# ariana-spalter/human-robot-gym

Hardware: AMD Instinct MI355X
Metric: env steps/sec (whole node), ReachHuman+shield 4096 envs (higher is better)
Workload: dtype f64

## Files before the change

### human-robot-gym_amd/csrc/hrgym_device.h

```cpp
#pragma once
#include <hip/hip_runtime.h>
#include <stdint.h>

#include "../../include/hrgym.h"
#include "../../include/hrgym_state.h"

#define NV HRG_NV
#define NARM HRG_NARM
#ifndef HRG_BOX
#define HRG_BOX 0
#endif
#ifndef HRG_LIFT
#define HRG_LIFT 0
#endif
#ifndef HRG_HANDOVER
#define HRG_HANDOVER 0
#endif
#ifndef HRG_STACK
#define HRG_STACK 0
#endif
#ifndef HRG_HULLS
#define HRG_HULLS 0
#endif
#ifndef HRG_HAMMER
#define HRG_HAMMER 0
#endif
#define HRG_BASE_TU (!HRG_BOX && !HRG_STACK && !HRG_HAMMER && !HRG_HULLS)
#define HRG_POSE_TABLE ((!HRG_BOX && !HRG_STACK && !HRG_HAMMER) || HRG_LIFT)
#define HRG_POSE_HCAP 0
#define HRG_POSE_SITE (6 * HRG_NHB)
#define HRG_POSE_ROOT (HRG_POSE_SITE + 3 * HRG_NHJ)
#define HRG_POSE_DIM (HRG_POSE_ROOT + 3)
#define NVT HRG_NVT
#if HRG_HAMMER
#define NVS HRG_NV_HAMMER
#define NCON_DYN HRG_NCON_DYN_HAMMER
#define HM_OB NV
#define HM_ON (NV + 6)
#define HM_OH (NV + 8)
#elif HRG_STACK
#define NVS HRG_NV_STACK
#define NCON_DYN HRG_NCON_DYN_STACK
#define NCUBE HRG_NCUBE
#elif HRG_BOX
#define NVS NVT
#define NCON_DYN HRG_NCON_DYN_BOX
#else
#define NVS NV
#define NCON_DYN HRG_NCON_DYN
#endif
#define BODY_BOX 100
#define DI __device__ __forceinline__
#ifndef HRG_MIN_WAVES
#define HRG_MIN_WAVES 4
#endif
#ifndef HRG_PHASE
#define HRG_PHASE __device__ __forceinline__
#endif
#define PH_DYNTERMS HRG_PHASE
#define PH_HUMAN HRG_PHASE
#define PH_SHIELD HRG_PHASE
#define PH_COLLIDE HRG_PHASE
#define PH_CLASSIFY HRG_PHASE
#define PH_DYNSTEP HRG_PHASE
#define HRG_PI 3.14159265358979323846
#define SIXTH (1.0 / 6.0)

#define GEOM_HUMAN0 HRG_NRCAP
#define GEOM_TABLE (HRG_NRCAP + HRG_NHB)
#define GEOM_FLOOR (GEOM_TABLE + 1)
#define GEOM_BOX (GEOM_FLOOR + 1)

#ifdef HRG_STAMPS
static __device__ unsigned long long g_stamps[32];
static __device__ unsigned long long g_stamps_slow[34];
static __device__ unsigned long long g_slow_thresh = ~0ull;
static __device__ unsigned long long g_envcyc[16384][3];
static __device__ unsigned long long g_envacc[16384][32];
__shared__ unsigned long long g_tbeg;
__shared__ unsigned long long g_acc[32];
__shared__ unsigned long long g_t0;
#define STAMP_NOW(var) do { __builtin_amdgcn_sched_barrier(0); asm volatile("s_memtime %0\n\ts_waitcnt lgkmcnt(0)" : "=s"(var) :: "memory"); __builtin_amdgcn_sched_barrier(0); } while (0)
#define STAMP_DECL
#define STAMP_INIT(lane) do { if ((lane) < 32) g_acc[lane] = 0; unsigned long long _t; STAMP_NOW(_t); g_t0 = _t; g_tbeg = _t; __syncthreads(); } while (0)
#define STAMP(k) do { unsigned long long _t; STAMP_NOW(_t); if (threadIdx.x == 0) { g_acc[k] += _t - g_t0; g_t0 = _t; } } while (0)
#define STAMP_FLUSH(lane)
#define COUNT(k, n) do { if (threadIdx.x == 0) g_acc[k] += (n); } while (0)
#define STAMP_FINAL(lane) do { __syncthreads(); if ((lane) < 32) atomicAdd(&g_stamps[lane], g_acc[lane]); { unsigned long long _te; STAMP_NOW(_te); if (_te - g_tbeg > g_slow_thresh) { if ((lane) < 32) atomicAdd(&g_stamps_slow[lane], g_acc[lane]); if ((lane) == 32) atomicAdd(&g_stamps_slow[32], 1ull); if ((lane) == 33) atomicAdd(&g_stamps_slow[33], _te - g_tbeg); } } if ((lane) < 32 && blockIdx.x < 16384) g_envacc[blockIdx.x][lane] = g_acc[lane]; if ((lane) == 0 && blockIdx.x < 16384) { unsigned long long _t; STAMP_NOW(_t); g_envcyc[blockIdx.x][0] = g_tbeg; g_envcyc[blockIdx.x][1] = _t; unsigned _hw, _xcc; asm volatile("s_getreg_b32 %0, hwreg(HW_REG_HW_ID)\n\ts_getreg_b32 %1, hwreg(HW_REG_XCC_ID)" : "=s"(_hw), "=s"(_xcc)); g_envcyc[blockIdx.x][2] = ((unsigned long long)_xcc << 32) | _hw; } } while (0)
#else
#define STAMP_DECL
#define STAMP_INIT(lane)
#define STAMP(k)
#define STAMP_FLUSH(lane)
#define COUNT(k, n)
#define STAMP_FINAL(lane)
#endif

struct DevModel {
  hrg_model_desc m;
  double Rbase[9];
  double Rq[NV][9];
  int32_t anc_mask[NV];
  int32_t hb_maxdepth;
  double sol_K, sol_Bd;
  double rcap_hl[HRG_NRCAP], hcap_hl[HRG_NHB];
  int32_t hb_njump;
  int32_t hb_jump[4][HRG_NHB];
  int32_t phase_mask;
  hrg_path brake_full;
  double brake_T, brake_ds;
  int32_t hc_n;
  int32_t hc_kind[HRG_NHCAP_MAX], hc_j1[HRG_NHCAP_MAX], hc_j2[HRG_NHCAP_MAX];
  double hc_th[HRG_NHCAP_MAX], hc_v[HRG_NHCAP_MAX], hc_a[HRG_NHCAP_MAX], hc_len[HRG_NHCAP_MAX];
  int32_t n_self;
  int32_t self_i[64], self_j[64];
  int32_t n_chk;
  int32_t chk_i[32], chk_j[32];
  hrg_clip_table clips;
  const double* pose_tab;
  const double* hull_dev;
  double hull_cen[HRG_NHULL][3];
  unsigned long long* mpr_fallback;
};

static inline void hull_centroids(const double* verts, const int32_t* off, double cen[HRG_NHULL][3]) {
  for (int h = 0; h < HRG_NHULL; h++) {
    double s[3] = {0, 0, 0};
    for (int i = off[h]; i < off[h + 1]; i++) for (int a = 0; a < 3; a++) s[a] += verts[3 * i + a];
    for (int a = 0; a < 3; a++) cen[h][a] = s[a] / (double)(off[h + 1] - off[h]);
  }
}

struct Contact {
  int32_t g1, g2, b1, b2;
  double dist, n[3], pos[3];
};

#define ROW_CON0 24
#define ROW_WELD0 (ROW_CON0 + 4 * NCON_DYN)
#if HRG_HAMMER
#define HROW_NFRIC 8
#define HROW_LIM0 9
#define HROW_NLIM 25
#define HROW_EQ0 27
#define HROW_CON0 36
#define HROW_NEQ 9
#define NROW 128
#elif HRG_STACK
#define SROW_WELD0 24
#define SROW_CON0 36
#define NROW HRG_NROW_STACK
#elif HRG_BOX && (HRG_HANDOVER || HRG_LIFT)
#define NROW (ROW_WELD0 + 6)
#else
#define NROW ROW_WELD0
#endif

struct GjkLds { double y[4][3], a[4][3], b[4][3], l[4], lam[4]; int ia[4], ib[4]; };
#define HRG_HULL_MPR (HRG_HULLS && (HRG_BOX || HRG_STACK || HRG_HAMMER))
#if HRG_HULL_MPR
struct MprLds { double v[5][3], a[5][3], b[5][3]; };
#endif
struct Lds {
  hrg_env_state st;
  double kR[NV][9], kp[NV][3], Sw[NV][3], Sv[NV][3], vw[NV][3], vv[NV][3];
  double M[NV * NV];
  double bias[NV], a0[NVS], Ma0[NVS], ctrl[NV], qacc[NVS], g[NVS], d[NVS];
#if HRG_BOX
  hrg_box_state bx;
  double bR[9];
  double bMr[9];
  double hand_q[4], hand_off[3];
  int palm_hit, palm_pad;
#if HRG_HANDOVER
  double hcap_keep[HRG_NHB][6];
#endif
#endif
  double act[NV];
  int acc_has_collision, acc_collision_type, acc_failsafe, acc_pad;
#if HRG_HAMMER
  hrg_hammer_state hm;
  double gR[2][9];
  double gc[HRG_HM_NGEOM][3];
  double nail_org[3], nail_axis[3];
  double Mb[64], fb[8];
  double Ihw[9], tauh[3];
  double nsG[(9 + 2 * NCON_DYN) * (10 + 2 * NCON_DYN) / 2];
  Contact con[NCON_DYN];
#elif HRG_STACK
  hrg_stack_state sk;
  Contact con[NCON_DYN];
#elif HRG_BOX
  Contact con[NCON_DYN];
#else
  Contact con[NCON_DYN];
#endif
  union {
    struct {
      double cq[NARM], cv[NARM], ca[NARM], qe[NARM];
      double scap[2][HRG_NSHIELD_RCAP][6];
      double rc[HRG_NSHIELD_RCAP][7];
      hrg_ltt cand;
    };
    struct {
      double F[NV][6];
    };
    struct {
      double hcap[HRG_NHB][6], rcapw[HRG_NRCAP][6];
      int hnear[HRG_NHB];
      double rcen[HRG_NRCAP][3];
#if HRG_HULL_MPR
      union { GjkLds gjk; MprLds mpr; };
#elif HRG_HULLS
      GjkLds gjk;
#endif
#if HRG_STACK
      double cR[NCUBE][9];
#endif
    };
#if HRG_HAMMER
    struct {
      double Jc[4 * NCON_DYN + HROW_NEQ][NVS + 1], rg[NROW], rh[NROW];
    };
#elif HRG_STACK
    struct {
      double Jc[4 * NCON_DYN][21], rg[NROW], rh[NROW];
      int con_ca[NCON_DYN], con_cb[NCON_DYN], con_rob[NCON_DYN + 1];
    };
#else
    struct {
      double Jc[4 * NCON_DYN + (HRG_LIFT ? 6 : 0)][NVS + 1], rg[NROW], rh[NROW];
    };
#endif
  };
};

#ifndef HRG_WG_WAVES
#define HRG_WG_WAVES 1
#endif
#if HRG_WG_WAVES > 1
__shared__ Lds g_Lw[HRG_WG_WAVES];
#define g_L (g_Lw[__builtin_amdgcn_readfirstlane((int)(threadIdx.x >> 6))])
#else
__shared__ Lds g_L;
#endif
DI int hrg_lane() { return (int)(threadIdx.x & 63u); }
#define HRG_FAIR_SLOTS (8 * 8 * 2 * 16 * 4 * 8)
struct StepOrder { int32_t* buf; int32_t n; int32_t parity; int32_t* fair; };
DI int hrg_env() { return (int)blockIdx.x * HRG_WG_WAVES + (int)(threadIdx.x >> 6); }
#define HRG_LAUNCH_DIMS(n) dim3(((n) + HRG_WG_WAVES - 1) / HRG_WG_WAVES), dim3(64 * HRG_WG_WAVES)

typedef const DevModel __attribute__((address_space(4)))* ModelPtr;
DI ModelPtr uniform_model(const DevModel* dm) {
  const unsigned long long a = (unsigned long long)dm;
  unsigned lo = __builtin_amdgcn_readfirstlane((unsigned)(a & 0xffffffffull));
  unsigned hi = __builtin_amdgcn_readfirstlane((unsigned)(a >> 32));
  asm volatile("" : "+s"(lo), "+s"(hi));
  return (ModelPtr)(((unsigned long long)hi << 32) | lo);
}

DI double fsqrt(double x) {
  const double y = __builtin_amdgcn_rsq(x);
  double g = x * y, h = 0.5 * y;
  const double r = __builtin_fma(-h, g, 0.5);
  g = __builtin_fma(g, r, g);
  h = __builtin_fma(h, r, h);
  g = __builtin_fma(__builtin_fma(-g, g, x), h, g);
  g = __builtin_fma(__builtin_fma(-g, g, x), h, g);
  return x > 0 ? g : 0.0;
}
DI void v3set(double* r, double a, double b, double c) { r[0] = a; r[1] = b; r[2] = c; }
template <class PA>
DI void v3cpy(double* r, PA a) { r[0] = a[0]; r[1] = a[1]; r[2] = a[2]; }
template <class PA, class PB>
DI void v3add(double* r, PA a, PB b) { r[0] = a[0] + b[0]; r[1] = a[1] + b[1]; r[2] = a[2] + b[2]; }
template <class PA, class PB>
DI void v3sub(double* r, PA a, PB b) { r[0] = a[0] - b[0]; r[1] = a[1] - b[1]; r[2] = a[2] - b[2]; }
template <class PA>
DI void v3scl(double* r, PA a, double s) { r[0] = a[0] * s; r[1] = a[1] * s; r[2] = a[2] * s; }
template <class PA, class PB>
DI void v3madd(double* r, PA a, PB b, double s) { r[0] = a[0] + b[0] * s; r[1] = a[1] + b[1] * s; r[2] = a[2] + b[2] * s; }
template <class PA, class PB>
DI double v3dot(PA a, PB b) { return a[0] * b[0] + a[1] * b[1] + a[2] * b[2]; }
template <class PA>
DI double v3norm(PA a) { return fsqrt(v3dot(a, a)); }
template <class PA, class PB>
DI void v3cross(double* r, PA a, PB b) {
  double x = a[1] * b[2] - a[2] * b[1], y = a[2] * b[0] - a[0] * b[2], z = a[0] * b[1] - a[1] * b[0];
  r[0] = x; r[1] = y; r[2] = z;
}
template <class PA, class PB>
DI void m3mulv(double* r, PA M, PB v) {
  double x = M[0] * v[0] + M[1] * v[1] + M[2] * v[2];
  double y = M[3] * v[0] + M[4] * v[1] + M[5] * v[2];
  double z = M[6] * v[0] + M[7] * v[1] + M[8] * v[2];
  r[0] = x; r[1] = y; r[2] = z;
}
template <class PA, class PB>
DI void m3mul(double* R, PA A, PB B) {
  double T[9];
#pragma unroll
  for (int i = 0; i < 3; i++)
#pragma unroll
    for (int j = 0; j < 3; j++) T[3 * i + j] = A[3 * i] * B[j] + A[3 * i + 1] * B[3 + j] + A[3 * i + 2] * B[6 + j];
#pragma unroll
  for (int i = 0; i < 9; i++) R[i] = T[i];
}
template <class PA>
DI void quat2mat(double* M, PA q) {
  double w = q[0], x = q[1], y = q[2], z = q[3];
  M[0] = 1 - 2 * (y * y + z * z); M[1] = 2 * (x * y - w * z); M[2] = 2 * (x * z + w * y);
  M[3] = 2 * (x * y + w * z); M[4] = 1 - 2 * (x * x + z * z); M[5] = 2 * (y * z - w * x);
  M[6] = 2 * (x * z - w * y); M[7] = 2 * (y * z + w * x); M[8] = 1 - 2 * (x * x + y * y);
}
template <class PA, class PB>
DI void quatmul(double* r, PA a, PB b) {
  double w = a[0] * b[0] - a[1] * b[1] - a[2] * b[2] - a[3] * b[3];
  double x = a[0] * b[1] + a[1] * b[0] + a[2] * b[3] - a[3] * b[2];
  double y = a[0] * b[2] - a[1] * b[3] + a[2] * b[0] + a[3] * b[1];
  double z = a[0] * b[3] + a[1] * b[2] - a[2] * b[1] + a[3] * b[0];
  r[0] = w; r[1] = x; r[2] = y; r[3] = z;
}
DI void sincos_small(double x, double* sn, double* cs) {
  const double k = rint(x * 6.36619772367581382433e-01);
  const double r = (x - k * 1.57079632673412561417e+00) - k * 6.07710050650619224932e-11;
  const double z = r * r;
  const double ps = r + r * z * (-1.66666666666666324348e-01 + z * (8.33333333332248946124e-03 + z * (-1.98412698298579493134e-04 +
                    z * (2.75573137070700676789e-06 + z * (-2.50507602534068634195e-08 + z * 1.58969099521155010221e-10)))));
  const double pc = 1.0 - 0.5 * z + z * z * (4.16666666666666019037e-02 + z * (-1.38888888888741095749e-03 + z * (2.48015872894767294178e-05 +
                    z * (-2.75573143513906633035e-07 + z * (2.08757232129817482790e-09 + z * -1.13596475577881948265e-11)))));
  const int q = ((int)k) & 3;
  const double s0 = (q & 1) ? pc : ps, c0 = (q & 1) ? ps : pc;
  *sn = (q & 2) ? -s0 : s0;
  *cs = ((q + 1) & 2) ? -c0 : c0;
}
template <class PA>
DI void axisangle2mat(double* M, PA ax, double ang) {
  double s, c;
  sincos_small(ang, &s, &c);
  double t = 1 - c, x = ax[0], y = ax[1], z = ax[2];
  M[0] = t * x * x + c; M[1] = t * x * y - s * z; M[2] = t * x * z + s * y;
  M[3] = t * x * y + s * z; M[4] = t * y * y + c; M[5] = t * y * z - s * x;
  M[6] = t * x * z - s * y; M[7] = t * y * z + s * x; M[8] = t * z * z + c;
}
DI double clampd(double x, double lo, double hi) { return x < lo ? lo : (x > hi ? hi : x); }

template <int CTRL, int ROW_MASK>
DI double dpp_f64(double v) {
  const long long b = __double_as_longlong(v);
  const int lo = __builtin_amdgcn_update_dpp(0, (int)(b & 0xffffffffLL), CTRL, ROW_MASK, 0xf, false);
  const int hi = __builtin_amdgcn_update_dpp(0, (int)(b >> 32), CTRL, ROW_MASK, 0xf, false);
  return __longlong_as_double(((long long)hi << 32) | (unsigned int)lo);
}
DI double wave_sum(double v) {
  v += dpp_f64<0xB1, 0xf>(v);
  v += dpp_f64<0x4E, 0xf>(v);
  v += dpp_f64<0x141, 0xf>(v);
  v += dpp_f64<0x140, 0xf>(v);
  v += dpp_f64<0x142, 0xa>(v);
  v += dpp_f64<0x143, 0xc>(v);
  const long long b = __double_as_longlong(v);
  const int lo = __builtin_amdgcn_readlane((int)(b & 0xffffffffLL), 63);
  const int hi = __builtin_amdgcn_readlane((int)(b >> 32), 63);
  return __longlong_as_double(((long long)hi << 32) | (unsigned int)lo);
}
DI double wave_max(double v) {
#pragma unroll
  for (int o = 32; o > 0; o >>= 1) { double t = __shfl_xor(v, o, 64); v = t > v ? t : v; }
  return v;
}
DI double row16_max(double v) {
  double t;
  t = dpp_f64<0xB1, 0xf>(v); v = t > v ? t : v;
  t = dpp_f64<0x4E, 0xf>(v); v = t > v ? t : v;
  t = dpp_f64<0x141, 0xf>(v); v = t > v ? t : v;
  t = dpp_f64<0x140, 0xf>(v); v = t > v ? t : v;
  return v;
}
#if HRG_WG_WAVES > 1
DI void wave_sync() { __builtin_amdgcn_fence(__ATOMIC_RELEASE, "workgroup"); __builtin_amdgcn_wave_barrier(); __builtin_amdgcn_fence(__ATOMIC_ACQUIRE, "workgroup"); }
#else
DI void wave_sync() { __syncthreads(); }
#endif

DI uint64_t mix64(uint64_t x) {
  x += 0x9E3779B97F4A7C15ULL;
  x = (x ^ (x >> 30)) * 0xBF58476D1CE4E5B9ULL;
  x = (x ^ (x >> 27)) * 0x94D049BB133111EBULL;
  return x ^ (x >> 31);
}
DI double rng_u01(uint64_t seed, uint64_t env, uint64_t episode, uint64_t stream, uint64_t idx) {
  uint64_t h = mix64(seed);
  h = mix64(h ^ (env * 0xD1B54A32D192ED03ULL));
  h = mix64(h ^ (episode * 0x8CB92BA72F3D8DD7ULL));
  h = mix64(h ^ (stream * 0xABC98388FB8FAC03ULL + idx));
  return (double)(h >> 11) * (1.0 / 9007199254740992.0);
}
// ... 486 lines not shown
```

### human-robot-gym_amd/csrc/hrgym_kernels.h

```cpp
#pragma once
#include "hrgym_device.h"
#if HRG_HULLS
#include "hrgym_hull.h"
#endif

DI void robot_chain_fk(const DevModel* __restrict__ dm_, int lane, bool shield_on) {
  const ModelPtr dm = uniform_model(dm_);
  Lds& L = g_L;
  double* sc = &L.rc[0][0];
  if (lane < 3 * NARM && (lane >= 2 * NARM || shield_on)) {
    const int cfg = lane / NARM, i = lane - NARM * cfg;
    const double q = cfg == 0 ? L.cq[i] : (cfg == 1 ? L.qe[i] : L.st.qpos[i]);
    double sn, cs;
    sincos_small(q, &sn, &cs);
    sc[2 * lane] = sn; sc[2 * lane + 1] = cs;
  }
  wave_sync();
  if (lane < 9 && (lane >= 6 || shield_on)) {
    const auto& m = dm->m;
    const int cfg = lane / 3, row = lane - 3 * cfg;
    double r0 = dm->Rbase[3 * row], r1 = dm->Rbase[3 * row + 1], r2 = dm->Rbase[3 * row + 2];
    double p = m.base_pos[row];
#pragma unroll 1
    for (int i = 0; i < NARM; i++) {
// ... 283 lines not shown
  Lds& L = g_L;
  hrg_env_state& s = L.st;
  const double* e = dm->pose_tab + f * HRG_POSE_DIM;
  const bool cap = lane < HRG_NHB, site = !cap && lane < HRG_NHB + HRG_NHJ;
  double y[6] = {0, 0, 0, 0, 0, 0};
  if (cap) {
    const double2* p = (const double2*)(e + HRG_POSE_HCAP + 6 * lane);
    const double2 a = p[0], b = p[1], d = p[2];
    y[0] = a.x; y[1] = a.y; y[2] = b.x; y[3] = b.y; y[4] = d.x; y[5] = d.y;
  } else if (site) {
    const double* p = e + HRG_POSE_SITE + 3 * (lane - HRG_NHB);
    y[0] = p[0]; y[1] = p[1]; y[2] = p[2];
  }
  const double __attribute__((address_space(4)))* ec = (const double __attribute__((address_space(4)))*)(e + HRG_POSE_ROOT);
  double R[9], o[3], x[3];
  quat2mat(R, s.human_rot_offset);
  v3add(o, s.human_pos_offset, ec);
  m3mulv(x, R, y);
  if (cap) {
    v3add(&L.hcap[lane][0], o, x);
    m3mulv(x, R, y + 3);
    v3add(&L.hcap[lane][3], o, x);
  } else if (site) v3add(L.st.human_site[lane - HRG_NHB], o, x);
  wave_sync();
}

DI void human_pose_fk(const DevModel* __restrict__ dm_, int lane, int clip, int at, int hold_body = -1, int hold_left = 0) {
  const ModelPtr dm = uniform_model(dm_);
#if HRG_POSE_TABLE
  (void)hold_body; (void)hold_left;
  human_pose_from_table(dm, lane, (int64_t)dm->clips.clip_offset[clip] + at);
#else
  Lds& L = g_L;
  hrg_env_state& s = L.st;
  const double* fr = dm->clips.frames + (dm->clips.clip_offset[clip] + at) * HRG_FRAME_DIM;
  double qbi[4], qa[4], c[3], mp[3], mq[4], q1[4];
  human_root(dm, clip, fr, c, qbi, qa);
  v3add(mp, c, s.human_pos_offset);
  quatmul(q1, s.human_rot_offset, qbi);
  quatmul(mq, q1, qa);
  human_fk_lanes(dm_, lane, mp, mq, fr + 7, hold_body, hold_left);
#endif
}

#if HRG_BOX || HRG_STACK || HRG_HAMMER
DI double loop_prop(ModelPtr dm, int64_t gid, int episode, int ai, int clip, int k, int speed) {
  double base = speed ? dm->clips.clip_loop_speed[clip][k % HRG_MAX_LOOP] : dm->clips.clip_loop_amp[clip][k % HRG_MAX_LOOP];
  if (k >= HRG_MAX_LOOP) base = speed ? dm->clips.clip_loop2_speed[clip][k - HRG_MAX_LOOP] : dm->clips.clip_loop2_amp[clip][k - HRG_MAX_LOOP];
  const double sf = speed ? dm->clips.clip_loop_speed_std[clip] : dm->clips.clip_loop_amp_std[clip];
  const double z = clampd(rng_gauss(dm->m.seed, (uint64_t)gid, (uint64_t)episode, STREAM_LOOP, (uint64_t)((ai * 2 * HRG_MAX_LOOP + k) * 2 + speed)), -3.0, 3.0);
  return base * exp(z * log(sf));
}
DI double layered_sines(ModelPtr dm, int64_t gid, int episode, int ai, int clip, int kfirst, int n, double t, double start) {
  static_assert(2 * HRG_MAX_LOOP <= 64, "one lane per loop property");
  const int lane = hrg_lane(), kk = lane % HRG_MAX_LOOP, sp = (lane / HRG_MAX_LOOP) & 1;
  const double mine = loop_prop(dm, gid, episode, ai, clip, kfirst + (kk < n ? kk : 0), sp);
  double sum = 0;
  for (int k = 0; k < n; k++) {
    const double A = __shfl(mine, k), S = __shfl(mine, HRG_MAX_LOOP + k);
    sum += A * sin((t - start) / (A / S)) + start;
  }
  return sum - start * (double)(n - 1);
}
#endif

PH_HUMAN void human_control(const DevModel* __restrict__ dm_, int lane, int64_t gid) {
  const ModelPtr dm = uniform_model(dm_);
  Lds& L = g_L;
  const auto& m = dm->m;
  hrg_env_state& s = L.st;
  int control_time = (int)floor((double)s.low_level_time / m.anim_step_length);
  int at = control_time - s.anim_start_time;
  int anim_index = s.anim_index, anim_start = s.anim_start_time;
  int clip = clip_of(dm, gid, s.episode, anim_index);
#if HRG_BOX
  if (m.task == HRG_TASK_INSPECTION) {
    hrg_box_state& bx = L.bx;
    const int classic = control_time - s.anim_start_time, k0 = dm->clips.clip_keyframes[clip][0], k1 = dm->clips.clip_keyframes[clip][1], len = dm->clips.clip_len[clip];
    int phase = bx.task_phase, nd = bx.n_delayed;
    at = classic;
    if (at > k0 && phase == HRG_PHASE_APPROACH) phase = HRG_PHASE_READY;
    if (phase == HRG_PHASE_READY) {
      const int nl = dm->clips.clip_n_loop[clip];
      double sum = 0;
      for (int k = 0; k < nl; k++) {
        const double A = loop_prop(dm, gid, s.episode, s.anim_index, clip, k, 0), S = loop_prop(dm, gid, s.episode, s.anim_index, clip, k, 1);
        sum += A * sin((double)(classic - k0) / (A / S)) + (double)k0;
      }
      at = (int)(sum - (double)k0 * (double)(nl - 1));
      nd = classic - at;
    } else at -= nd;
    if (at > k1) phase = HRG_PHASE_RETREAT;
    if (at >= len - 1) { phase = HRG_PHASE_COMPLETE; at = len - 1; }
    if (at < 0) at = 0;
    wave_sync();
    bx.task_phase = phase; bx.n_delayed = nd;
    if (lane < 3) bx.target[lane] = dm->clips.clip_target_pos[clip][lane] + s.human_pos_offset[lane];
  }
  int hold_body = -1, hold_left = 0;
#if HRG_HANDOVER
  if (m.task == HRG_TASK_HANDOVER_H2R) {
    hrg_box_state& bx = L.bx;
    const int classic = at, k0 = dm->clips.clip_keyframes[clip][0], k1 = dm->clips.clip_keyframes[clip][1], len = dm->clips.clip_len[clip];
    int phase = bx.task_phase, nd = bx.n_delayed, nd2 = bx.n_delayed2;
    if (at > k0 && phase == HRG_PHASE_APPROACH) phase = HRG_PHASE_PRESENT;
    else if ((double)at > (double)k0 + (double)(k1 - k0) / 2.0 && phase == HRG_PHASE_PRESENT) {
      at = (int)layered_sines(dm, gid, s.episode, s.anim_index, clip, 0, dm->clips.clip_n_loop[clip], (double)classic, (double)(k0 + k1) / 2.0);
      nd = classic - at; nd2 = 0;
    } else if (phase == HRG_PHASE_WAIT) {
      at = classic - nd;
      if (at >= k1) at = (int)layered_sines(dm, gid, s.episode, s.anim_index, clip, HRG_MAX_LOOP, dm->clips.clip_n_loop2[clip], (double)at, (double)k1);
      nd2 = classic - at;
    } else if (phase == HRG_PHASE_RETREAT) at -= nd2;
    if (at >= len - 1) { phase = HRG_PHASE_COMPLETE; at = len - 1; }
    if (at < 0) at = 0;
    wave_sync();
    bx.task_phase = phase; bx.n_delayed = nd; bx.n_delayed2 = nd2;
    hold_left = dm->clips.clip_holding_hand[clip];
    hold_body = m.meas_body[hold_left ? m.site_lhand : m.site_rhand];
  }
  if (m.task == HRG_TASK_HANDOVER_R2H) {
    hrg_box_state& bx = L.bx;
    const int classic = at, k0 = dm->clips.clip_keyframes[clip][0], k1 = dm->clips.clip_keyframes[clip][1], len = dm->clips.clip_len[clip];
    int phase = bx.task_phase, nd = bx.n_delayed;
    if (at > k0 && phase == HRG_R2H_APPROACH) phase = HRG_R2H_REACH_OUT;
    if ((double)at > (double)k0 + (double)(k1 - k0) / 2.0 && phase == HRG_R2H_REACH_OUT) {
      at = (int)layered_sines(dm, gid, s.episode, s.anim_index, clip, 0, dm->clips.clip_n_loop[clip], (double)classic, (double)(k0 + k1) / 2.0);
      nd = classic - at;
    }
    if (phase == HRG_R2H_RETREAT) at -= nd;
    if (at >= len - 1) { phase = HRG_R2H_COMPLETE; at = len - 1; }
    if (at < 0) at = 0;
    wave_sync();
    bx.task_phase = phase; bx.n_delayed = nd;
    hold_left = dm->clips.clip_holding_hand[clip];
    hold_body = m.meas_body[hold_left ? m.site_lhand : m.site_rhand];
  }
#endif
#endif
#if HRG_STACK
  {
    hrg_stack_state& sk = L.sk;
    const int classic = at, len = dm->clips.clip_len[clip];
    const int k0 = dm->clips.clip_stack_keyframes[clip][0], k2 = dm->clips.clip_stack_keyframes[clip][2], k4 = dm->clips.clip_stack_keyframes[clip][4];
    int phase = sk.task_phase, nd0 = sk.n_delayed[0], nd1 = sk.n_delayed[1];
    if (phase == HRG_STK_APPROACH && at > k0) phase = HRG_STK_PLACE_FIRST;
    else if (phase == HRG_STK_WAIT_FOR_SECOND) {
      if (at >= k2) at = (int)layered_sines(dm, gid, s.episode, s.anim_index, clip, 0, dm->clips.clip_n_loop[clip], (double)classic, (double)k2);
      nd0 = classic - at; nd1 = 0;
    } else if (phase == HRG_STK_PLACE_THIRD) at = classic - nd0;
    else if (phase == HRG_STK_WAIT_FOR_FOURTH) {
      at = classic - nd0;
      if (at >= k4) at = (int)layered_sines(dm, gid, s.episode, s.anim_index, clip, HRG_MAX_LOOP, dm->clips.clip_n_loop2[clip], (double)at, (double)k4);
      nd1 = classic - at;
    } else if (phase == HRG_STK_RETREAT) at = classic - nd1;
    if (at >= len - 1) { phase = HRG_STK_COMPLETE; at = len - 1; }
    if (at < 0) at = 0;
    wave_sync();
    sk.task_phase = phase; sk.n_delayed[0] = nd0; sk.n_delayed[1] = nd1;
  }
#endif
#if HRG_HAMMER
  {
    hrg_hammer_state& hm = L.hm;
    const int classic = at, len = dm->clips.clip_len[clip];
    const double k0 = (double)dm->clips.clip_keyframes[clip][0], mid = 0.5 * (k0 + (double)dm->clips.clip_keyframes[clip][1]);
    int phase = hm.task_phase, nd = hm.n_delayed;
    if (phase == HRG_HM_APPROACH && (double)at > k0) phase = HRG_HM_PRESENT;
    else if (phase == HRG_HM_PRESENT && (double)at > mid) {
      at = (int)layered_sines(dm, gid, s.episode, s.anim_index, clip, 0, dm->clips.clip_n_loop[clip], (double)classic, mid);
      nd = classic - at;
    } else if (phase == HRG_HM_RETREAT) at -= nd;
    if (at >= len - 1) { phase = HRG_HM_COMPLETE; at = len - 1; }
    if (at < 0) at = 0;
    wave_sync();
    hm.task_phase = phase; hm.n_delayed = nd;
  }
#endif
#if HRG_LIFT
  if (m.task == HRG_TASK_LIFTING) {
    const int len = dm->clips.clip_len[clip];
    const bool complete = at >= len - 1;
    if (complete) at = len - 1;
    if (at < 0) at = 0;
    wave_sync();
    if (complete) L.bx.task_phase = HRG_PHASE_COMPLETE;
  }
#endif
  if (at > dm->clips.clip_len[clip] - 1) {
    anim_index = (anim_index + 1) % m.n_anim_ids;
    at = 0;
    anim_start = control_time;
    clip = clip_of(dm, gid, s.episode, anim_index);
  }
  s.anim_index = anim_index; s.anim_start_time = anim_start; s.animation_time = at;
#if HRG_BOX
  human_pose_fk(dm_, lane, clip, at, hold_body, hold_left);
#else
  human_pose_fk(dm_, lane, clip, at);
#endif
}

PH_SHIELD void shield_step(const DevModel* __restrict__ dm_, int lane, int e, double* __restrict__ dbg_r, double* __restrict__ dbg_h, int32_t* __restrict__ dbg_nh) {
  const ModelPtr dm = uniform_model(dm_);
  Lds& L = g_L;
  const auto& m = dm->m;
  hrg_env_state& s = L.st;
  const double dt = m.timestep, t = s.time;
  const bool shield_on = m.shield_type != HRG_SHIELD_OFF;
  const bool have_vel = s.n_meas >= 1 && t > s.meas_prev_t;
  if (lane < NARM) { L.cq[lane] = s.des_q[lane]; L.cv[lane] = s.des_v[lane]; L.ca[lane] = s.des_a[lane]; }
  wave_sync();
  int use_cand = 0;
  if (s.new_goal) {
    double nq = 0, nv = 0, na = 0;
    if (lane < NARM) ltt_eval(&s.ltt, lane, s.path_s, &nq, &nv, &na);
    const bool bad = lane < NARM && fabs(na) > m.a_max_ltt[lane];
    if (!__any(bad)) {
      use_cand = 1;
      double tj = 0;
      LttTail tail;
      tail.n0 = 0; tail.v = tail.sg = tail.Dm = tail.vm = tail.w = 0;
      if (lane < NARM) {
        ltt_plan_joint(&L.cand, lane, nq, nv, na, s.new_goal_q[lane], m.v_max_ltt[lane], m.a_max_ltt[lane], m.j_max_ltt[lane], &tail);
        for (int i = 0; i < HRG_LTT_NSEG; i++) tj += L.cand.dur[lane][i];
      }
      const double Tall = wave_max(tj);
      L.cand.T = Tall;
      if (m.ltt_time_sync && lane < NARM) ltt_sync_joint(&L.cand, lane, Tall, m.a_max_ltt[lane], m.j_max_ltt[lane], tail);
    }
    wave_sync();
  }
  STAMP(10);
  const hrg_ltt* Lp = use_cand ? &L.cand : &s.ltt;
  const double ps = use_cand ? 0.0 : s.path_s, pv = s.path_v, pa = s.path_a;
  hrg_path fs2;
  double s1, v1, a1, se, Tb;
  const bool pfl = m.shield_type == HRG_SHIELD_PFL, steady = pv == 1.0 && pa == 0.0;
  if (steady) { s1 = ps + dt; v1 = 1.0; a1 = 0.0; }
  else {
    hrg_path rec;
    path_plan(&rec, ps, pv, pa, 1.0, m.path_amax, m.path_jmax);
    path_eval(&rec, dt, 1.0, &s1, &v1, &a1);
  }
  double ve_fs = m.failsafe_sdot;
  if (pfl) {
    double q_, d1_ = 0, d2_;
    if (lane < NARM) ltt_eval(Lp, lane, s1, &q_, &d1_, &d2_);
    const double vc = wave_sum(lane < NARM ? fabs(d1_) * m.pfl_reach[lane] : 0.0);
    ve_fs = vc > m.pfl_v_safe ? m.pfl_v_safe / vc : 1.0;
  }
  if (steady && !pfl) {
    fs2.s0 = s1; fs2.v0 = 1.0; fs2.a0 = 0.0; fs2.k = 0.0;
    for (int a = 0; a < 3; a++) { fs2.dur[a] = dm->brake_full.dur[a]; fs2.jerk[a] = dm->brake_full.jerk[a]; }
    Tb = dm->brake_T;
    se = s1 + dm->brake_ds;
  } else {
    double ve_, ae;
    path_plan(&fs2, s1, v1, a1, ve_fs, m.path_amax, m.path_jmax);
    Tb = path_total(&fs2);
    path_eval(&fs2, Tb, ve_fs, &se, &ve_, &ae);
  }
  s1 = uniform_f64(s1); v1 = uniform_f64(v1); a1 = uniform_f64(a1); se = uniform_f64(se); Tb = uniform_f64(Tb);
  fs2.s0 = uniform_f64(fs2.s0); fs2.v0 = uniform_f64(fs2.v0); fs2.a0 = uniform_f64(fs2.a0); fs2.k = uniform_f64(fs2.k);
  for (int a = 0; a < 3; a++) { fs2.dur[a] = uniform_f64(fs2.dur[a]); fs2.jerk[a] = uniform_f64(fs2.jerk[a]); }
  STAMP(11);
  if (shield_on && lane < NARM) {
    double qn, q1, q2, qv;
    ltt_eval2(Lp, lane, s1, se, &qn, &q1, &q2, &qv);
    L.qe[lane] = qv;
    s.des_q[lane] = qn; s.des_v[lane] = q1 * v1; s.des_a[lane] = q1 * a1 + q2 * v1 * v1;
  }
  wave_sync();
  STAMP(12);
  robot_chain_fk(dm_, lane, shield_on);
  STAMP(13);
  int safe = 1;
  if (shield_on) {
    const double sdiff = se - ps;
    double rc_hl = 0;
    if (lane < HRG_NSHIELD_RCAP) {
      const int c = lane;
      double d[3], l1, l2;
      v3sub(d, &L.scap[0][c][0], &L.scap[1][c][0]); l1 = v3norm(d);
      v3sub(d, &L.scap[0][c][3], &L.scap[1][c][3]); l2 = v3norm(d);
      for (int a = 0; a < 6; a++) L.rc[c][a] = 0.5 * (L.scap[0][c][a] + L.scap[1][c][a]);
      L.rc[c][6] = m.scap_r[c] + m.secure_radius + 0.5 * (l1 > l2 ? l1 : l2) + m.scap_alpha[c] * sdiff * sdiff / 8.0;
      double hv[3];
      for (int a = 0; a < 3; a++) hv[a] = 0.5 * (L.rc[c][3 + a] - L.rc[c][a]);
      rc_hl = fsqrt(v3dot(hv, hv));
      L.scap[0][c][0] = rc_hl;
      if (dbg_r) for (int a = 0; a < 7; a++) dbg_r[((size_t)e * HRG_NSHIELD_RCAP + c) * 7 + a] = L.rc[c][a];
    }
    wave_sync();
    double rbl[3], rbh[3];
    {
      double bl[3], bh[3];
      if (lane < HRG_NSHIELD_RCAP) {
        const double rr = L.rc[lane][6];
        for (int a = 0; a < 3; a++) { const double p1 = L.rc[lane][a], p2 = L.rc[lane][3 + a]; bl[a] = (p1 < p2 ? p1 : p2) - rr; bh[a] = (p1 > p2 ? p1 : p2) + rr; }
      } else for (int a = 0; a < 3; a++) { bl[a] = 1e300; bh[a] = -1e300; }
      for (int a = 0; a < 3; a++) { rbh[a] = lane_value<0>(row16_max(bh[a])); rbl[a] = -lane_value<0>(row16_max(-bl[a])); }
    }
    const int nh = dm->hc_n;
    int mdl = -1;
    double c1[3] = {0, 0, 0}, c2[3] = {0, 0, 0}, r = 0, hc[3] = {0, 0, 0}, hl = 0;
    bool near_robot = false;
    if (lane < nh) {
      const int kind = dm->hc_kind[lane], j1 = dm->hc_j1[lane], j2 = dm->hc_j2[lane];
      const double Td = dt + Tb + m.delay;
      if (kind == 0) {
        double va[3], vb[3];
        const double idt = have_vel ? 1.0 / (t - s.meas_prev_t) : 0.0;
        for (int a = 0; a < 3; a++) {
          va[a] = (s.human_site[j1][a] - s.meas_prev[j1][a]) * idt;
          vb[a] = (s.human_site[j2][a] - s.meas_prev[j2][a]) * idt;
        }
        const double base = 0.5 * dm->hc_a[lane] * Td * Td + m.meas_err_pos + m.meas_err_vel * Td;
        const double r1 = v3norm(va) * Td * 0.5 + base, r2 = v3norm(vb) * Td * 0.5 + base;
        v3madd(c1, s.human_site[j1], va, 0.5 * Td);
        v3madd(c2, s.human_site[j2], vb, 0.5 * Td);
        r = (r1 > r2 ? r1 : r2) + dm->hc_th[lane];
        mdl = 0;
      } else if (kind == 2) {
        v3cpy(c1, s.human_site[j1]);
        v3cpy(c2, s.human_site[j1]);
        r = dm->hc_len[lane] + dm->hc_th[lane] + m.meas_err_pos + dm->hc_v[lane] * Td;
        mdl = 2;
      } else {
        v3cpy(c1, s.human_site[j1]);
        v3cpy(c2, s.human_site[j2]);
        r = dm->hc_th[lane] + m.meas_err_pos + dm->hc_v[lane] * Td;
        mdl = kind == 1 ? 1 : 2;
      }
      double hh[3];
      for (int a = 0; a < 3; a++) { hc[a] = 0.5 * (c1[a] + c2[a]); hh[a] = 0.5 * (c2[a] - c1[a]); }
      hl = fsqrt(v3dot(hh, hh));
      double d2b = 0;
      for (int a = 0; a < 3; a++) { const double ee = hc[a] < rbl[a] ? rbl[a] - hc[a] : (hc[a] > rbh[a] ? hc[a] - rbh[a] : 0.0); d2b += ee * ee; }
      near_robot = d2b <= (hl + r + 1e-9) * (hl + r + 1e-9);
      if (dbg_h) {
        double* o = dbg_h + ((size_t)e * HRG_NHCAP_MAX + lane) * 7;
        o[0] = c1[0]; o[1] = c1[1]; o[2] = c1[2]; o[3] = c2[0]; o[4] = c2[1]; o[5] = c2[2]; o[6] = r;
      }
    }
    if (dbg_nh && lane == 0) dbg_nh[e] = nh;
    bool all_hit = true;
#pragma unroll 1
    for (int mm = 0; mm < 3 && all_hit; mm++) {
      if (mm == 0 && !have_vel) continue;
      const bool mine = mdl == mm && near_robot;
      bool hit = false;
      if (__any(mine)) {
#pragma unroll 1
        for (int c = 0; c < HRG_NSHIELD_RCAP; c++) {
          bool close = false;
          const double rr = L.rc[c][6] + r;
          if (mine) {
            double rcn[3], dc[3];
            for (int a = 0; a < 3; a++) rcn[a] = 0.5 * (L.rc[c][a] + L.rc[c][3 + a]);
            v3sub(dc, rcn, hc);
            const double reach = L.scap[0][c][0] + hl + rr + 1e-9;
            close = !(v3dot(dc, dc) > reach * reach);
          }
          if (!__any(close)) continue;
          if (close) { double x1[3], x2[3]; if (seg_seg(&L.rc[c][0], &L.rc[c][3], c1, c2, x1, x2) < rr * rr) hit = true; }
          if (__any(hit)) break;
        }
      }
      all_hit = __any(hit);
    }
    safe = !all_hit;
  }
  wave_sync();
  STAMP(14);
  for (int k = lane; k < HRG_NHJ * 3; k += 64) (&s.meas_prev[0][0])[k] = (&s.human_site[0][0])[k];
  s.meas_prev_t = t;
  if (s.n_meas < 2) s.n_meas = s.n_meas + 1;
  if (safe) {
    if (use_cand) {
      double* dst = (double*)&s.ltt;
      const double* src = (const double*)&L.cand;
      for (int k = lane; k < (int)(sizeof(hrg_ltt) / sizeof(double)); k += 64) dst[k] = src[k];
      s.new_goal = 0;
    }
    s.path_s = s1; s.path_v = v1; s.path_a = a1;
    s.safe_path = fs2;
  } else {
    const double k = s.safe_path.k + 1.0;
    s.safe_path.k = k;
    double ns, nv, na;
    const hrg_path spc = s.safe_path;
    const double vend = pfl ? path_vend(&spc) : m.failsafe_sdot;
    path_eval(&s.safe_path, k * dt, vend, &ns, &nv, &na);
    if (use_cand && s.path_v <= vend + 1e-9 && fabs(s.path_a) <= 1e-9) {
      const double adv = ns - s.path_s;
      double* dst = (double*)&s.ltt;
      const double* src = (const double*)&L.cand;
      for (int q = lane; q < (int)(sizeof(hrg_ltt) / sizeof(double)); q += 64) dst[q] = src[q];
      s.new_goal = 0;
      ns = adv;
      hrg_path sp;
      path_plan(&sp, ns, nv, na, vend, m.path_amax, m.path_jmax);
      s.safe_path = sp;
    }
    s.path_s = ns; s.path_v = nv; s.path_a = na;
  }
  s.is_safe = safe;
  wave_sync();
  if (lane < NARM && !(shield_on && safe)) {
    double qq, q1, q2;
    ltt_eval(&s.ltt, lane, s.path_s, &qq, &q1, &q2);
    s.des_q[lane] = qq; s.des_v[lane] = q1 * s.path_v; s.des_a[lane] = q1 * s.path_a + q2 * s.path_v * s.path_v;
  }
  wave_sync();
  STAMP(15);
}

DI void shield_reset(const DevModel* __restrict__ , int lane) {
  Lds& L = g_L;
  hrg_env_state& s = L.st;
  if (lane < NARM) {
    const double q = s.qpos[lane];
    s.ltt.q0[lane] = q; s.ltt.qT[lane] = q;
    s.des_q[lane] = q; s.new_goal_q[lane] = q; s.goal_qpos[lane] = q;
  }
  s.is_safe = 1;
}

#if HRG_STACK || HRG_HAMMER || HRG_LIFT
#define BB_TIE 1e-9
struct BBContact { double pos[3], n[3], dist; };
#define BB_WORK 152
DI int box_box2(const double* pa, const double* Ra, const double* ha, const double* pb, const double* Rb, const double* hb, BBContact* out, double* T) {
  double (*A)[3] = (double (*)[3])(T + 72), (*B)[3] = (double (*)[3])(T + 81), (*C)[3] = (double (*)[3])(T + 90), (*AC)[3] = (double (*)[3])(T + 99);
  double t[3], ta[3], tb[3];
  v3sub(t, pb, pa);
  for (int i = 0; i < 3; i++) for (int k = 0; k < 3; k++) { A[i][k] = Ra[3 * k + i]; B[i][k] = Rb[3 * k + i]; }
  for (int i = 0; i < 3; i++) { ta[i] = v3dot(t, A[i]); tb[i] = v3dot(t, B[i]); for (int j = 0; j < 3; j++) { C[i][j] = v3dot(A[i], B[j]); AC[i][j] = fabs(C[i][j]); } }
  double sf = -1e300, se = -1e300;
  int bf = 0, be = -1;
  for (int i = 0; i < 3; i++) {
    const double s_ = fabs(ta[i]) - (ha[i] + hb[0] * AC[i][0] + hb[1] * AC[i][1] + hb[2] * AC[i][2]);
    if (s_ > 0) return 0;
    if (s_ > sf + BB_TIE) { sf = s_; bf = i; }
  }
  for (int j = 0; j < 3; j++) {
    const double s_ = fabs(tb[j]) - (hb[j] + ha[0] * AC[0][j] + ha[1] * AC[1][j] + ha[2] * AC[2][j]);
    if (s_ > 0) return 0;
    if (s_ > sf + BB_TIE) { sf = s_; bf = 3 + j; }
  }
#pragma unroll 1
  for (int ij = 0; ij < 9; ij++) {
    const int i = ij / 3, j = ij - 3 * i, i1 = (i + 1) % 3, i2 = (i + 2) % 3, j1 = (j + 1) % 3, j2 = (j + 2) % 3;
    const double l2 = 1.0 - C[i][j] * C[i][j];
    if (l2 < 1e-12) continue;
    const double l = fsqrt(l2);
    const double tl = ta[i2] * C[i1][j] - ta[i1] * C[i2][j];
    const double s_ = (fabs(tl) - (ha[i1] * AC[i2][j] + ha[i2] * AC[i1][j] + hb[j1] * AC[i][j2] + hb[j2] * AC[i][j1])) / l;
    if (s_ > 0) return 0;
    if (s_ > se + BB_TIE) { se = s_; be = ij; }
  }
  if (be >= 0 && se * 1.05 > sf) {
    const int i = be / 3, j = be - 3 * i;
    double n[3], pA[3], pB[3], d[3];
    v3cross(n, A[i], B[j]);
    v3scl(n, n, 1.0 / v3norm(n));
    if (v3dot(n, t) < 0) v3scl(n, n, -1.0);
    v3cpy(pA, pa); v3cpy(pB, pb);
    for (int k = 0; k < 3; k++) {
      if (k != i) v3madd(pA, pA, A[k], (v3dot(n, A[k]) > 0 ? 1.0 : -1.0) * ha[k]);
      if (k != j) v3madd(pB, pB, B[k], (v3dot(n, B[k]) > 0 ? -1.0 : 1.0) * hb[k]);
    }
    v3sub(d, pB, pA);
    const double uaub = C[i][j], q1 = v3dot(A[i], d), q2 = -v3dot(B[j], d), den = 1.0 - uaub * uaub;
    const double al = (q1 + uaub * q2) / den, be_ = (uaub * q1 + q2) / den;
    double xa[3], xb[3];
    v3madd(xa, pA, A[i], al);
    v3madd(xb, pB, B[j], be_);
    for (int k = 0; k < 3; k++) out[0].pos[k] = 0.5 * (xa[k] + xb[k]);
    v3cpy(out[0].n, n);
    out[0].dist = se;
    return 1;
  }
  const bool refA = bf < 3;
  const int r = refA ? bf : bf - 3, r1 = (r + 1) % 3, r2 = (r + 2) % 3;
  double (*Rf)[3] = (double (*)[3])(T + 108), (*In)[3] = (double (*)[3])(T + 117);
  double pr[3], pi_[3];
  for (int a = 0; a < 3; a++) for (int k = 0; k < 3; k++) { Rf[a][k] = refA ? A[a][k] : B[a][k]; In[a][k] = refA ? B[a][k] : A[a][k]; }
  for (int k = 0; k < 3; k++) { pr[k] = refA ? pa[k] : pb[k]; pi_[k] = refA ? pb[k] : pa[k]; }
  const double* hr = refA ? ha : hb;
  const double* hi = refA ? hb : ha;
  const double sg = refA ? (ta[r] >= 0 ? 1.0 : -1.0) : (tb[r] >= 0 ? -1.0 : 1.0);
  double nr[3], cr[3], ci[3];
  v3scl(nr, Rf[r], sg);
  v3madd(cr, pr, nr, hr[r]);
  int k = 0;
  double best = -1;
  for (int q = 0; q < 3; q++) { const double c_ = fabs(v3dot(In[q], nr)); if (c_ > best) { best = c_; k = q; } }
  const int k1 = (k + 1) % 3, k2 = (k + 2) % 3;
  const double si = v3dot(In[k], nr) > 0 ? -1.0 : 1.0;
  v3madd(ci, pi_, In[k], si * hi[k]);
  const double hu = hr[r1], hv = hr[r2];
  const double S1[4] = {1, -1, -1, 1}, S2[4] = {1, 1, -1, -1};
  double *vu = T + 126, *vv = T + 130, *vd = T + 134;
  for (int q = 0; q < 4; q++) {
    double x[3], d[3];
    v3madd(x, ci, In[k1], S1[q] * hi[k1]);
    v3madd(x, x, In[k2], S2[q] * hi[k2]);
    v3sub(d, x, cr);
    vu[q] = v3dot(d, Rf[r1]); vv[q] = v3dot(d, Rf[r2]); vd[q] = v3dot(d, nr);
  }
  for (int q = 0; q < 24; q++) T[48 + q] = 1.0;
  auto offer = [&](int idx, double u, double v, double dpt) { if (dpt < 0) { T[idx] = u; T[24 + idx] = v; T[48 + idx] = dpt; } };
  for (int q = 0; q < 4; q++)
    if (fabs(vu[q]) <= hu && fabs(vv[q]) <= hv) offer(q, vu[q], vv[q], vd[q]);
  {
    double d0[3];
    v3sub(d0, ci, cr);
    const double c0u = v3dot(d0, Rf[r1]), c0v = v3dot(d0, Rf[r2]), c0d = v3dot(d0, nr);
    const double e1u = hi[k1] * v3dot(In[k1], Rf[r1]), e1v = hi[k1] * v3dot(In[k1], Rf[r2]), e1d = hi[k1] * v3dot(In[k1], nr);
    const double e2u = hi[k2] * v3dot(In[k2], Rf[r1]), e2v = hi[k2] * v3dot(In[k2], Rf[r2]), e2d = hi[k2] * v3dot(In[k2], nr);
    const double det = e1u * e2v - e1v * e2u;
    if (fabs(det) > 1e-12 * hu * hv)
      for (int q = 0; q < 4; q++) {
        const double pu = S1[q] * hu - c0u, pv = S2[q] * hv - c0v;
        const double al = (pu * e2v - pv * e2u) / det, be_ = (e1u * pv - e1v * pu) / det;
        if (fabs(al) <= 1 && fabs(be_) <= 1) offer(4 + q, S1[q] * hu, S2[q] * hv, c0d + al * e1d + be_ * e2d);
      }
  }
#pragma unroll 1
  for (int q = 0; q < 4; q++) {
    const int q1 = (q + 1) & 3;
    const double du = vu[q1] - vu[q], dv = vv[q1] - vv[q], dd = vd[q1] - vd[q];
#pragma unroll 1
    for (int e = 0; e < 4; e++) {
      const double lim = (e & 1) ? -1.0 : 1.0;
      if (e < 2) {
        if (fabs(du) < 1e-14) continue;
        const double tt = (lim * hu - vu[q]) / du, w = vv[q] + tt * dv;
        if (tt > 0 && tt < 1 && fabs(w) < hv) offer(8 + 4 * q + e, lim * hu, w, vd[q] + tt * dd);
      } else {
        if (fabs(dv) < 1e-14) continue;
        const double tt = (lim * hv - vv[q]) / dv, w = vu[q] + tt * du;
        if (tt > 0 && tt < 1 && fabs(w) < hu) offer(8 + 4 * q + e, w, lim * hv, vd[q] + tt * dd);
      }
    }
  }
  int pick[4], np_ = 0;
  const double eps2 = 1e-12 * (hu * hu + hv * hv);
  {
    int arg = -1;
    double bd = 0;
#pragma unroll 1
    for (int q = 0; q < 24; q++) { const double dq = T[48 + q]; if (dq < 0 && (arg < 0 || dq < bd - BB_TIE)) { arg = q; bd = dq; } }
    if (arg >= 0) pick[np_++] = arg;
  }
  if (np_ == 1) {
    int arg = -1;
    double bestv = eps2;
    const double u0 = T[pick[0]], v0 = T[24 + pick[0]];
#pragma unroll 1
    for (int q = 0; q < 24; q++) {
      if (!(T[48 + q] < 0)) continue;
      const double du = T[q] - u0, dv = T[24 + q] - v0, val = du * du + dv * dv;
      if (val > bestv * (1 + 1e-9)) { arg = q; bestv = val; }
    }
    if (arg >= 0) pick[np_++] = arg;
  }
  if (np_ == 2) {
    const double u0 = T[pick[0]], v0 = T[24 + pick[0]], lu = T[pick[1]] - u0, lv = T[24 + pick[1]] - v0, epsc = fsqrt(eps2 * (lu * lu + lv * lv));
    int argp = -1, argn = -1;
    double bp = epsc, bn = epsc;
#pragma unroll 1
    for (int q = 0; q < 24; q++) {
      if (!(T[48 + q] < 0)) continue;
      const double cr_ = lu * (T[24 + q] - v0) - lv * (T[q] - u0);
      if (cr_ > bp * (1 + 1e-9)) { argp = q; bp = cr_; }
      if (-cr_ > bn * (1 + 1e-9)) { argn = q; bn = -cr_; }
    }
    if (argp >= 0) pick[np_++] = argp;
    if (argn >= 0) pick[np_++] = argn;
  }
  for (int z = 0; z < np_; z++) {
    const double u = T[pick[z]], v = T[24 + pick[z]], dpt = T[48 + pick[z]];
    for (int a = 0; a < 3; a++) {
      out[z].pos[a] = cr[a] + u * Rf[r1][a] + v * Rf[r2][a] + 0.5 * dpt * nr[a];
      out[z].n[a] = refA ? nr[a] : -nr[a];
    }
    out[z].dist = dpt;
  }
  return np_;
}
DI int box_box(const double* pa, const double* Ra, const double* pb, const double* Rb, const double* h, BBContact* out, double* T) { return box_box2(pa, Ra, h, pb, Rb, h, out, T); }
#endif
#if HRG_HULLS && (HRG_STACK || HRG_HAMMER)
DI int mpr_link_box(const DevModel* __restrict__ dm_, int g, const double* bR, const double* bp, const double* bh, double& depth, double* n, double* pos) {
  const ModelPtr dm = uniform_model(dm_);
  Lds& L = g_L;
  const auto& m = dm->m;
  const int lb = m.rcap_body[g];
  const double* R = lb < 0 ? dm_->Rbase : L.kR[lb];
  const double* p = lb < 0 ? dm_->m.base_pos : L.kp[lb];
  const HullRef H = {dm_->hull_dev + 3 * m.hull_off[g], m.hull_off[g + 1] - m.hull_off[g], R, p};
  double hc[3];
  m3mulv(hc, R, dm_->hull_cen[g]);
  v3add(hc, hc, p);
  const int r = mpr_hull_box_wave(H, hc, bR, bp, bh, depth, n, pos);
  if (r == MPR_NOT_CONVERGED && hrg_lane() == 0) atomicAdd(dm_->mpr_fallback, 1ull);
  return r;
}
#endif
#if HRG_STACK

DI void collide_cubes(const DevModel* __restrict__ dm_, int lane, int* base_io) {
  const ModelPtr dm = uniform_model(dm_);
  Lds& L = g_L;
  const auto& m = dm->m;
  hrg_stack_state& sk = L.sk;
  int base = *base_io;
  const uint64_t lt = lane == 0 ? 0ull : (~0ull >> (64 - lane));
  if (lane < NCUBE) { double Rm[9]; quat2mat(Rm, sk.quat[lane]); for (int a = 0; a < 9; a++) L.cR[lane][a] = Rm[a]; }
  wave_sync();
  const double hb[3] = {m.box_half[0], m.box_half[1], m.box_half[2]};
  const double circ2 = hb[0] * hb[0] + hb[1] * hb[1] + hb[2] * hb[2];
  bool f0a = false, f1a = false, f0b = false, f1b = false;
#pragma unroll 1
  for (int round = 0; round < 4; round++) {
    Contact c;
    c.g1 = c.g2 = c.b1 = c.b2 = 0; c.dist = 0; v3set(c.n, 0, 0, 1); v3set(c.pos, 0, 0, 0);
    bool hit = false;
    if (round == 0 || round == 3) {
      const bool second = round == 3;
      const int cb = lane / HRG_NRCAP, i = lane - cb * HRG_NRCAP;
      bool near = false;
      if (lane < NCUBE * HRG_NRCAP && m.rcap_body[i] >= 0) {
        double dc[3];
        for (int a = 0; a < 3; a++) dc[a] = 0.5 * (L.rcapw[i][a] + L.rcapw[i][3 + a]) - sk.pos[cb][a];
        const double reach = dm->rcap_hl[i] + m.rcap_r[i] + fsqrt(circ2) + 1e-9;
        near = v3dot(dc, dc) <= reach * reach;
      }
      if (__any(near) && near) {
        double cs[3], cbp[3];
        const double e2 = seg_box(&L.rcapw[i][0], &L.rcapw[i][3], sk.pos[cb], L.cR[cb], hb, cs, cbp);
        double dd = fsqrt(e2), dist = dd - m.rcap_r[i];
        if (dist < 0) {
          double s2[3], b2[3];
          const bool two = dd > 1e-9 && cap_box_two(&L.rcapw[i][0], &L.rcapw[i][3], sk.pos[cb], L.cR[cb], hb, m.rcap_r[i], cs, cbp, second ? 1 : 0, s2, b2);
          if (two) { v3cpy(cs, s2); v3cpy(cbp, b2); double dv[3]; v3sub(dv, cbp, cs); dd = v3norm(dv); dist = dd - m.rcap_r[i]; }
          hit = two || !second;
          if (dd > 1e-9) { v3sub(c.n, cbp, cs); v3scl(c.n, c.n, 1.0 / dd); }
          else {
            double loc[3], rel[3], best = 1e300;
            int ax = 0;
            v3sub(rel, cs, sk.pos[cb]);
            for (int a = 0; a < 3; a++) { loc[a] = L.cR[cb][a] * rel[0] + L.cR[cb][3 + a] * rel[1] + L.cR[cb][6 + a] * rel[2]; if (hb[a] - fabs(loc[a]) < best) { best = hb[a] - fabs(loc[a]); ax = a; } }
            const double sg = loc[ax] >= 0 ? -1.0 : 1.0;
            for (int a = 0; a < 3; a++) c.n[a] = sg * L.cR[cb][3 * a + ax];
            dist = -best - m.rcap_r[i];
          }
          v3madd(c.pos, cs, c.n, m.rcap_r[i] + 0.5 * dist);
          c.g1 = i; c.g2 = GEOM_BOX + cb; c.b1 = m.rcap_body[i]; c.b2 = BODY_BOX + cb; c.dist = dist;
        }
      }
#if HRG_HULLS
      if (m.robot_hulls) {
        const bool link = lane < NCUBE * HRG_NRCAP && i < HRG_NHULL;
        if (second && link) hit = false;
        uint64_t todo = second ? 0ull : __ballot(hit && link);
// ... 667 lines not shown
```

Baseline: 4.497 million.

## Compact near human capsules and spread capsule pairs across all wave lanes

```diff
diff --git a/human-robot-gym_amd/csrc/hrgym_device.h b/human-robot-gym_amd/csrc/hrgym_device.h
--- a/human-robot-gym_amd/csrc/hrgym_device.h
+++ b/human-robot-gym_amd/csrc/hrgym_device.h
@@ -86,6 +86,11 @@
 #define STAMP(k) do { unsigned long long _t; STAMP_NOW(_t); if (threadIdx.x == 0) { g_acc[k] += _t - g_t0; g_t0 = _t; } } while (0)
 #define STAMP_FLUSH(lane)
 #define COUNT(k, n) do { if (threadIdx.x == 0) g_acc[k] += (n); } while (0)
+#if HRG_HAMMER
+#define STAMP_SHIELD(k)
+#else
+#define STAMP_SHIELD(k) STAMP(k)
+#endif
 #define STAMP_FINAL(lane) do { __syncthreads(); if ((lane) < 32) atomicAdd(&g_stamps[lane], g_acc[lane]); { unsigned long long _te; STAMP_NOW(_te); if (_te - g_tbeg > g_slow_thresh) { if ((lane) < 32) atomicAdd(&g_stamps_slow[lane], g_acc[lane]); if ((lane) == 32) atomicAdd(&g_stamps_slow[32], 1ull); if ((lane) == 33) atomicAdd(&g_stamps_slow[33], _te - g_tbeg); } } if ((lane) < 32 && blockIdx.x < 16384) g_envacc[blockIdx.x][lane] = g_acc[lane]; if ((lane) == 0 && blockIdx.x < 16384) { unsigned long long _t; STAMP_NOW(_t); g_envcyc[blockIdx.x][0] = g_tbeg; g_envcyc[blockIdx.x][1] = _t; unsigned _hw, _xcc; asm volatile("s_getreg_b32 %0, hwreg(HW_REG_HW_ID)\n\ts_getreg_b32 %1, hwreg(HW_REG_XCC_ID)" : "=s"(_hw), "=s"(_xcc)); g_envcyc[blockIdx.x][2] = ((unsigned long long)_xcc << 32) | _hw; } } while (0)
 #else
 #define STAMP_DECL
@@ -93,6 +98,7 @@
 #define STAMP(k)
 #define STAMP_FLUSH(lane)
 #define COUNT(k, n)
+#define STAMP_SHIELD(k)
 #define STAMP_FINAL(lane)
 #endif
 
diff --git a/human-robot-gym_amd/csrc/hrgym_kernels.h b/human-robot-gym_amd/csrc/hrgym_kernels.h
--- a/human-robot-gym_amd/csrc/hrgym_kernels.h
+++ b/human-robot-gym_amd/csrc/hrgym_kernels.h
@@ -609,6 +609,7 @@
       } else for (int a = 0; a < 3; a++) { bl[a] = 1e300; bh[a] = -1e300; }
       for (int a = 0; a < 3; a++) { rbh[a] = lane_value<0>(row16_max(bh[a])); rbl[a] = -lane_value<0>(row16_max(-bl[a])); }
     }
+    STAMP_SHIELD(29);
     const int nh = dm->hc_n;
     int mdl = -1;
     double c1[3] = {0, 0, 0}, c2[3] = {0, 0, 0}, r = 0, hc[3] = {0, 0, 0}, hl = 0;
@@ -652,26 +653,41 @@
       }
     }
     if (dbg_nh && lane == 0) dbg_nh[e] = nh;
+    STAMP_SHIELD(31);
+    int* const vnear = (int*)&L.scap[1][0][0];
+    static_assert(sizeof(int) * HRG_NHCAP_MAX <= sizeof(double) * HRG_NSHIELD_RCAP * 6, "the near list has to fit scap[1]");
+    const uint64_t lt = lane == 0 ? 0ull : (~0ull >> (64 - lane));
     bool all_hit = true;
 #pragma unroll 1
     for (int mm = 0; mm < 3 && all_hit; mm++) {
       if (mm == 0 && !have_vel) continue;
       const bool mine = mdl == mm && near_robot;
+      const uint64_t nearmask = __ballot(mine);
       bool hit = false;
-      if (__any(mine)) {
+      if (nearmask) {
+        if (mine) vnear[__popcll(nearmask & lt)] = lane;
+        wave_sync();
+        const int npairs = HRG_NSHIELD_RCAP * __popcll(nearmask);
 #pragma unroll 1
-        for (int c = 0; c < HRG_NSHIELD_RCAP; c++) {
+        for (int base = 0; base < npairs; base += 64) {
+          const int q = base + lane;
+          const bool valid = q < npairs;
+          const int k = valid ? q / HRG_NSHIELD_RCAP : 0, c = valid ? q - k * HRG_NSHIELD_RCAP : 0;
+          const int src = vnear[k];
+          double pc1[3], pc2[3], phc[3];
+          for (int a = 0; a < 3; a++) { pc1[a] = __shfl(c1[a], src, 64); pc2[a] = __shfl(c2[a], src, 64); phc[a] = 0.5 * (pc1[a] + pc2[a]); }
+          const double pr = __shfl(r, src, 64), phl = __shfl(hl, src, 64);
           bool close = false;
-          const double rr = L.rc[c][6] + r;
-          if (mine) {
+          const double rr = L.rc[c][6] + pr;
+          if (valid) {
             double rcn[3], dc[3];
             for (int a = 0; a < 3; a++) rcn[a] = 0.5 * (L.rc[c][a] + L.rc[c][3 + a]);
-            v3sub(dc, rcn, hc);
-            const double reach = L.scap[0][c][0] + hl + rr + 1e-9;
+            v3sub(dc, rcn, phc);
+            const double reach = L.scap[0][c][0] + phl + rr + 1e-9;
             close = !(v3dot(dc, dc) > reach * reach);
           }
           if (!__any(close)) continue;
-          if (close) { double x1[3], x2[3]; if (seg_seg(&L.rc[c][0], &L.rc[c][3], c1, c2, x1, x2) < rr * rr) hit = true; }
+          if (close) { double x1[3], x2[3]; if (seg_seg(&L.rc[c][0], &L.rc[c][3], pc1, pc2, x1, x2) < rr * rr) hit = true; }
           if (__any(hit)) break;
         }
       }
```

Result: no change. 4.516 million (median of 6 runs) (+0.4%).
